# HKU-BAL/ClairS-TO

Measured on AMD Instinct MI355X. Metric: candidate sites/sec (pileup-tensor + AFF/NEG inference) at 1/2/4/8 MI355X, higher is better.
Workload: dtype f32; 1 GPU; ONT 50x synthetic pileups, SNV (K=4), 1M-site job cut into 4096-site chunks (BASELINE.json configs[1]); step = featurize(AFF+NEG) + CvT + BiGRU + posterior on one chunk; batch=4096, chunks_resident_per_gpu=16, min_bq_aff=20, pack_bytes_per_chunk=28614435, parallelism=sites sharded, 1 rank/GPU, weights=seeded random init (no pretrained weights offline)

## Files before the change

### clairs_to_amd/csrc/cvt_block.h

```cpp
#pragma once
#include "cvt_gemm.h"

namespace cto {

__host__ __device__ constexpr int emb_ps(int cin) { return cin > 0 ? ((cin - 4 + 15) / 16) * 16 + 4 : 0; }
__host__ __device__ constexpr int emb_kch(int cin) { return (3 * emb_ps(cin) + 15) / 16; }

template <int C, int W, int WKV, int TS, bool FOLD = false, int ECIN = 0>
struct CvtBlockGeom {
    static_assert(!FOLD || C <= 64, "folding pays only where C <= dim_head");
    static constexpr int R = TS * W, RKV = TS * WKV;
    static constexpr int MT = (R + 15) / 16, MTKV = (RKV + 15) / 16;
    static constexpr int AW = FOLD ? C : 64;
    static constexpr int RS = C + 4, QS = AW + 4, HC = (4 * C < 128 ? 4 * C : 128), US = HC + 4;
    static constexpr int KV_FLOATS = FOLD ? 0 : MTKV * 16 * QS;
    static constexpr int OFF_Y = 0;
    static constexpr int OFF_YKV = OFF_Y + MT * 16 * RS;
    static constexpr int OFF_Q = OFF_YKV + MTKV * 16 * RS;
    static constexpr int OFF_K = OFF_Q + MT * 16 * QS;
    static constexpr int OFF_V = OFF_K + KV_FLOATS;
    static constexpr int OFF_END = OFF_V + KV_FLOATS;
    static constexpr int SCRATCH = OFF_END - OFF_YKV;
    static constexpr int U_FLOATS = MT * 16 * US;
    static constexpr int emb_floats(int cin) { return (MT * 32 + 4) * emb_ps(cin); }
    static constexpr int TOTAL_BLK = OFF_END + (U_FLOATS > SCRATCH ? U_FLOATS - SCRATCH : 0);
    static constexpr int TOTAL_EMB = FOLD && ECIN > 0 ? OFF_YKV + emb_floats(ECIN) : 0;
    static constexpr int TOTAL = TOTAL_BLK > TOTAL_EMB ? TOTAL_BLK : TOTAL_EMB;
    static constexpr size_t LDS_BYTES = size_t(TOTAL) * sizeof(float);
    static constexpr int TMP_FLOATS = OFF_END - OFF_Q;
    static constexpr int ALIAS = TOTAL - OFF_YKV;
    static constexpr int KCH1 = (W * RS + 15) / 16;
    static constexpr bool HEAD_OK = (TS == 16) && (64 + head_lds_floats(6) <= ALIAS);
};

// ... 49 lines not shown
                                                const BPreS<ColOwn<N>::NTW>& pre,
                                                f32x4 (&acc)[MSplit<MTx, ColOwn<N>::MSPLIT>::MTG][ColOwn<N>::NTW], int j, int kg) {
    using S = MSplit<MTx, ColOwn<N>::MSPLIT>;
    constexpr int NTW = ColOwn<N>::NTW;
    const float* A0 = A + sp.mbase * 16 * lda;
    if (ColOwn<N>::MSPLIT == 1 || sp.mcount == S::MTG) {
        gemm_lds_split<S::MTG, NTW, KCH, F16>(A0, lda, klo, wrow, pre, acc, j, kg);
    } else if constexpr (S::LAST > 0) {
        if (sp.mcount == S::LAST) {
            f32x4 (&sub)[S::LAST][NTW] = reinterpret_cast<f32x4 (&)[S::LAST][NTW]>(acc);
            gemm_lds_split<S::LAST, NTW, KCH, F16>(A0, lda, klo, wrow, pre, sub, j, kg);
        }
    }
}

template <int C, int W, int WKV, int TS, bool FOLD = false, int ECIN = 0>
__host__ __device__ constexpr int cvt_blocks_per_cu() {
    using G = CvtBlockGeom<C, W, WKV, TS, FOLD, ECIN>;
    return G::LDS_BYTES * 3 <= 160 * 1024 && !FOLD ? 3 : (G::LDS_BYTES * 2 <= 160 * 1024 ? 2 : 1);
}

template <int N>
__device__ __forceinline__ float rowN_sum(float v) {
    static_assert(N == 4 || N == 8 || N == 16, "a quad, half a DPP row or a DPP row");
    v += dpp_mov<0xB1>(v);
    v += dpp_mov<0x4E>(v);
    if constexpr (N >= 8) v += dpp_mov<0x141>(v);
    if constexpr (N >= 16) v += dpp_mov<0x140>(v);
    return v;
}

template <int C, int W, int WKV, int TS, int CIN, bool HEAD, int SPLIT = 0, bool FOLD = false>
__global__ __launch_bounds__(CVT_BLOCK_THREADS, (2 * cvt_blocks_per_cu<C, W, WKV, TS, FOLD, FOLD ? CIN : 0>())) void k_cvt_block(float* __restrict__ h, CvtStageParams sp,
                                                                                                                  HeadTailParams hp, int heads, int B) {
    using G = CvtBlockGeom<C, W, WKV, TS, FOLD, FOLD ? CIN : 0>;
    static_assert(!FOLD || SPLIT == 0, "the folded matrices exist in fp32 only");
    constexpr bool SP = SPLIT != 0, F16 = SPLIT == 1;
    static_assert(!SP || (C % 64 == 0 && MT_EXACT<C, W, WKV, TS>()), "split GEMMs: 32-wide k chunks, 16-byte LayerNorm pieces, no pad rows");
    using WPtr = std::conditional_t<SP, const unsigned short*, const float*>;
    static_assert(CIN == 0 || G::emb_floats(CIN) <= G::ALIAS, "stage input tile does not fit the free LDS");
    static_assert(!HEAD || G::HEAD_OK, "classifier tail needs a 16-site tile and room for its scratch");
    static_assert(G::MT * 16 * G::RS <= G::TMP_FLOATS, "LayerNorm staging tile does not fit the q|k|v region");
    constexpr int NT = CVT_BLOCK_THREADS, NWV = CVT_WAVES;
    constexpr int R = G::R, MT = G::MT, MTKV = G::MTKV, RKV = G::RKV, RS = G::RS, QS = G::QS, HC = G::HC, US = G::US, AW = G::AW;
    static_assert(C % 16 == 0 && C <= 128 && NT % C == 0, "channel count must be 16, 32, 64 or 128");
    using OC = ColOwn<C>;
    using OQ = ColOwn<AW>;
    using OKV = ColOwn<128>;
    using OF = ColOwn<HC>;
    constexpr int MGC = MSplit<MT, OC::MSPLIT>::MTG, MGQ = MSplit<MT, OQ::MSPLIT>::MTG, MGF = MSplit<MT, OF::MSPLIT>::MTG;
    constexpr int NTC = OC::NTW, NTF = OF::NTW;
    static_assert(OQ::NTW == 1 && OKV::NTW == 1 && OKV::MSPLIT == 1, "q / kv tiles: one column tile per wave");
    extern __shared__ __attribute__((aligned(16))) float smem[];
    float* sy = smem + G::OFF_Y;
    float* sykv = smem + G::OFF_YKV;
    float* sq = smem + G::OFF_Q;
    float* sk = smem + G::OFF_K;
    float* sv = smem + G::OFF_V;
    float* stmp = smem + G::OFF_Q;
    float* su = smem + G::OFF_YKV;

    const int tid = threadIdx.x, lane = tid & 63, wave = tid >> 6, j = lane & 15, kg = lane >> 4;
    const TileSpan spc = tile_span<C, MT>(wave), spq = tile_span<AW, MT>(wave), spf = tile_span<HC, MT>(wave);
    const int site0 = blockIdx.x * TS;
    const int nsite = min(TS, B - site0);
    const int rows_valid = nsite * W;
    const int inner = heads * AW;
    float* hg = h + int64_t(site0) * W * C;
    int nstamp = 0;
    long long* const prof = sp.blk[0].prof;
    auto stamp = [&]() { if (prof && blockIdx.x == 0 && tid == 0 && nstamp < 250) prof[nstamp++] = clock64(); };
    stamp();
    const CvtBlockParams& pe = sp.blk[0];


    constexpr int KE_ = CIN > 0 ? emb_kch(CIN) : 1;
    const float* we_r[NTC];
    BPre<NTC> pre_e;
    if constexpr (CIN > 0) {
#pragma unroll
        for (int nt = 0; nt < NTC; ++nt) we_r[nt] = pe.wembp + int64_t(spc.tile0 + nt) * (KE_ * FRAG_CS) + 4 * lane;
        pre_e = prefetch_b<NTC, KE_>(we_r);
// ... 158 lines not shown
                if (mt < spc.mcount) {
#pragma unroll
                    for (int r = 0; r < 4; ++r) sy[((spc.mbase + mt) * 16 + 4 * kg + r) * RS + col] = acc_e[mt][nt][r] + bv;
                }
        }
        lds_barrier();
        for (int i = tid; i < (MTKV * 16 - RKV) * RS; i += NT) sykv[RKV * RS + i] = 0.f;
        layer_norm(sy, sy, pe.lng, pe.lnb, std::false_type{});
        lds_barrier();
    }

    f32x4 acc_f[MGC][NTC];
    for (int bi = 0; bi < sp.nblk; ++bi) {
    const CvtBlockParams& p = sp.blk[bi];
    stamp();
    f32x4 acc_o[MGC][NTC];
#pragma unroll
    for (int nt = 0; nt < NTC; ++nt) {
        const int col = (spc.tile0 + nt) * 16 + j;
        const float bv = p.bo[col];
#pragma unroll
        for (int mt = 0; mt < MGC; ++mt) {
            const int row0 = (spc.mbase + (mt < spc.mcount ? mt : 0)) * 16 + 4 * kg;
            if (bi == 0) {
#pragma unroll
                for (int r = 0; r < 4; ++r) acc_o[mt][nt][r] = sy[(row0 + r) * RS + col] + bv;
            } else {
#pragma unroll
                for (int r = 0; r < 4; ++r) acc_o[mt][nt][r] = acc_f[mt][nt][r] + bv;
            }
        }
    }
    layer_norm(sy, stmp, p.n0g, p.n0b, std::false_type{});
    lds_barrier();
    stamp();

#if CTO_CVT_ABL != 2
    {
        constexpr int NSLOT = NT / C;
        constexpr int PG = NSLOT > TS ? NSLOT / TS : 1;
        constexpr int SL = PG > 1 ? TS : NSLOT, NIT = (TS + SL - 1) / SL;
        constexpr int WQ = (W + PG - 1) / PG, WK = (WKV + PG - 1) / PG;
        const int c = tid % C, slot = tid / C, pg = slot / SL, s0 = slot - pg * SL;
        const int wlo = pg * WQ, whi = min(W, wlo + WQ), klo = pg * WK, khi = min(WKV, klo + WK);
        const float q0 = p.dwq[c * 3], q1 = p.dwq[c * 3 + 1], q2 = p.dwq[c * 3 + 2];
        const float k0 = p.dwkv[c * 3], k1 = p.dwkv[c * 3 + 1], k2 = p.dwkv[c * 3 + 2];
// ... 27 lines not shown
                    if constexpr (SP) put_split1<F16>(sykv + (s * WKV + wo) * RS, C, c, (d - km) * ki * kw + kb);
                    else sykv[(s * WKV + wo) * RS + c] = (d - km) * ki * kw + kb;
                }
            }
        }
    }
#endif
    lds_barrier();

    stamp();
    auto frag = [&](const float* w, const unsigned short* ws, int tile, int kch, int c0) -> WPtr {
        if constexpr (SP) return ws + (int64_t(tile) * kch + c0) * SPLIT_CS + 8 * lane;
        else return w + (int64_t(tile) * kch + c0) * FRAG_CS + 4 * lane;
    };
    constexpr int KD = SP ? 32 : 16;
    auto q_rows = [&](int hh, WPtr (&wr)[1]) { wr[0] = frag(p.wq, p.wq_s, hh * (AW / 16) + spq.tile0, C / KD, 0); };
    auto o_rows = [&](int hh, WPtr (&wr)[NTC]) {
#pragma unroll
        for (int nt = 0; nt < NTC; ++nt) wr[nt] = frag(p.wo, p.wo_s, spc.tile0 + nt, inner / KD, hh * (AW / KD));
    };
    auto w1_rows = [&](int cc, WPtr (&wr)[NTF]) {
#pragma unroll
        for (int nt = 0; nt < NTF; ++nt) wr[nt] = frag(p.w1, p.w1_s, cc * (HC / 16) + spf.tile0 + nt, C / KD, 0);
    };
    auto w2_rows = [&](int cc, WPtr (&wr)[NTC]) {
#pragma unroll
        for (int nt = 0; nt < NTC; ++nt) wr[nt] = frag(p.w2, p.w2_s, spc.tile0 + nt, 4 * C / KD, cc * (HC / KD));
    };
    WPtr wq_r[1];
    q_rows(0, wq_r);
    auto pre_q = prefetch_b<1, C / KD>(wq_r);
    for (int hh = 0; hh < heads; ++hh) {
        const int wn = wave & 3;
        WPtr wkv1_r[1] = {frag(p.wkv, p.wkv_s, (wave < 4 ? 0 : inner / 16) + hh * 4 + wn, C / KD, 0)};
        decltype(prefetch_b<1, C / KD>(wkv1_r)) pre_kv1;
        if constexpr (!FOLD) pre_kv1 = prefetch_b<1, C / KD>(wkv1_r);
        {
            f32x4 aq[MGQ][1];
#pragma unroll
            for (int mt = 0; mt < MGQ; ++mt) aq[mt][0] = f32x4{0.f, 0.f, 0.f, 0.f};
            if constexpr (SP) gemm_span_split<64, MT, C / 32, F16>(spq, sy, RS, C, wq_r, pre_q, aq, j, kg);
            else gemm_span<AW, MT, C / 16>(spq, sy, RS, wq_r, pre_q, aq, j, kg);
// ... 68 lines not shown
                }
            }
        }
#endif
        if (hh + 1 < heads) {
            q_rows(hh + 1, wq_r);
            pre_q = prefetch_b<1, C / KD>(wq_r);
        }
        lds_barrier();
        stamp();
        if constexpr (SP) gemm_span_split<C, MT, 2, F16>(spc, sq, QS, 64, wo_r, pre_o, acc_o, j, kg);
        else gemm_span<C, MT, AW / 16>(spc, sq, QS, wo_r, pre_o, acc_o, j, kg);
        lds_barrier();
        stamp();
    }

    WPtr w1_r[NTF];
    w1_rows(0, w1_r);
    auto pre_w1 = prefetch_b<NTF, C / KD>(w1_r);

#pragma unroll
    for (int nt = 0; nt < NTC; ++nt) {
        const int col = (spc.tile0 + nt) * 16 + j;
        const float bv = p.b2[col];
#pragma unroll
        for (int mt = 0; mt < MGC; ++mt) {
            if (mt < spc.mcount) {
#pragma unroll
                for (int r = 0; r < 4; ++r) stmp[((spc.mbase + mt) * 16 + 4 * kg + r) * RS + col] = acc_o[mt][nt][r];
            }
#pragma unroll
            for (int r = 0; r < 4; ++r) acc_f[mt][nt][r] = acc_o[mt][nt][r] + bv;
        }
    }
    lds_barrier();

    stamp();
    layer_norm(stmp, sy, p.n1g, p.n1b, std::bool_constant<SP>{});
    lds_barrier();
    stamp();

    for (int cc = 0; cc < 4 * C / HC; ++cc) {
        WPtr w2_r[NTC];
        w2_rows(cc, w2_r);
        const auto pre_w2 = prefetch_b<NTC, HC / KD>(w2_r);
        {
            f32x4 au[MGF][NTF];
#pragma unroll
            for (int mt = 0; mt < MGF; ++mt)
#pragma unroll
// ... 82 lines not shown
```

### clairs_to_amd/csrc/models.hip

```cpp
#include <cmath>
#include <cstdlib>
#include <cstring>
#include <map>
#include <memory>
#include <string>
#include <vector>
#include "common.h"
#include "nn_kernels.h"
#include "cvt_block.h"

using namespace cto;

int launch_gru_layer1(hipStream_t s, const float* x, const float* Wf, const float* bias, float* out, int64_t B);
int launch_gru_layer1_raw(hipStream_t s, const int16_t* x_raw, const int32_t* site_info, int which, int min_rescale_cov, const float* Wf,
                          const float* bias, float* out, int64_t B);
int launch_gru_layer2_fc1_split(hipStream_t s, const float* x, const void* Wp, const float* bias, const void* Fp, float* fc1_part,
                                int64_t B, bool f16, const float* scale5);
int launch_gru_layer1_split(hipStream_t s, const float* x, const void* Wp, const float* bias, float* out, int64_t B, bool f16,
                            const float* scale5);
int launch_gru_layer2_fc1(hipStream_t s, const float* x, const float* Wf, const float* bias, const float* fc1f, float* fc1_part, int64_t B);


struct cto_weights {
    std::map<std::string, std::vector<float>> t;
// ... 23 lines not shown
        if (rc != CTO_OK) return rc;
        CTO_HIP(hipMemcpy(p, v.data(), v.size() * sizeof(float), hipMemcpyHostToDevice));
        *out = static_cast<float*>(p);
        return CTO_OK;
    }
};

struct HeadDev {
    float *w1 = nullptr, *b1 = nullptr;
    float* w1p = nullptr;
    float *w2 = nullptr, *b2 = nullptr;
    float *w3 = nullptr, *b3 = nullptr;
    int k1 = 0;
};

struct BlockDev {
    float *n0g, *n0b, *dwq, *bnq, *wq, *dwkv, *bnkv, *wkv, *wo, *bo, *n1g, *n1b, *w1, *b1, *w2, *b2;
    float *wq_f = nullptr, *wkv_f = nullptr, *wo_f = nullptr, *w1_f = nullptr, *w2_f = nullptr;
    float *mq_f = nullptr, *mo_f = nullptr;
    float *wq_s = nullptr, *wkv_s = nullptr, *wo_s = nullptr, *w1_s = nullptr, *w2_s = nullptr;
};

struct StageDev {
    int cin, c, win, w, wkv, heads, inner;
    float *wemb, *bemb, *lng, *lnb;
    float* wembp = nullptr;
    std::vector<BlockDev> blocks;
};

}

struct cto_model {
    int device = -1;
    int kind = 0;
// ... 3 lines not shown
    float *gb1 = nullptr, *gb2 = nullptr;
    float *gw1f = nullptr, *gw2f = nullptr, *f1f = nullptr;
    float *gw1_split = nullptr, *gw2_split = nullptr, *f1_split = nullptr;
    bool split_f16 = false;
    float split_sc1[5] = {1.f, 1.f, 1.f, 1.f, 1.f}, split_sc2[5] = {1.f, 1.f, 1.f, 1.f, 1.f};
    int cvt_split = 0;
    HeadDev head;
    int64_t macs = 0;
    int64_t ws_B = 0;
    std::vector<void*> ws_ptrs;
    float* b_xexp = nullptr;
    int64_t xexp_B = 0;
    bool fuse_blocks = true;
    bool fuse_embed = true;
    bool fuse_head = true;
    bool fold = true;
    bool prof = false;
    bool prof_all = false;
    std::vector<std::pair<hipEvent_t, hipEvent_t>> prof_ev;
    std::vector<std::pair<hipEvent_t, hipEvent_t>> prof_ev1;
    int64_t prof_macs = 0;
    float *b_h = nullptr, *b_t = nullptr, *b_yq = nullptr, *b_ykv = nullptr, *b_q = nullptr, *b_kv = nullptr,
          *b_o = nullptr, *b_u = nullptr, *b_slab = nullptr, *b_h2 = nullptr;
    ~cto_model() {
        if (b_xexp) (void)hipFree(b_xexp);
        for (void* p : ws_ptrs) (void)hipFree(p);
        for (auto& e : prof_ev) { (void)hipEventDestroy(e.first); (void)hipEventDestroy(e.second); }
        for (auto& e : prof_ev1) { (void)hipEventDestroy(e.first); (void)hipEventDestroy(e.second); }
    }
};

// ... 168 lines not shown
        return rc;
    return launch_head(m, s, m->b_slab, S, B, logits);
}

struct RawIn { const int16_t* x; const int32_t* site_info; int which, min_rescale_cov; };

struct BlockExtra {
    const float* xin = nullptr;
    const RawIn* raw = nullptr;
    const StageDev* st = nullptr;
    const HeadDev* head = nullptr;
    float* logits = nullptr;
    int n_out = 0;
};

template <int C, int W, int WKV, int TS, int CIN, bool HEAD, int SPLIT = 0, bool FOLD = false>
int launch_cvt_block(hipStream_t s, float* h, const BlockDev* blocks, int nblk, int heads, int64_t B, const BlockExtra& ex) {
    using G = CvtBlockGeom<C, W, WKV, TS, FOLD, FOLD ? CIN : 0>;
    static_assert(G::LDS_BYTES <= 160 * 1024, "fused CvT block does not fit the 160 KB LDS of a gfx950 CU");
    static bool attr_set = false;
    if (!attr_set) {
        CTO_HIP(hipFuncSetAttribute(reinterpret_cast<const void*>(&k_cvt_block<C, W, WKV, TS, CIN, HEAD, SPLIT, FOLD>),
                                    hipFuncAttributeMaxDynamicSharedMemorySize, int(G::LDS_BYTES)));
        attr_set = true;
    }
    static long long* prof_buf = nullptr;
    static const bool prof_on = [] { const char* e = getenv("CTO_BLOCK_PROF"); return e && e[0] == '1'; }();
    if (prof_on && !prof_buf) CTO_HIP(hipMalloc(reinterpret_cast<void**>(&prof_buf), 256 * sizeof(long long)));
    if (prof_on) CTO_HIP(hipMemsetAsync(prof_buf, 0, 256 * sizeof(long long), s));
    CvtStageParams sp{};
    sp.nblk = nblk;
    for (int i = 0; i < nblk; ++i) {
        const BlockDev& b = blocks[i];
        if (FOLD) CTO_REQUIRE(b.mq_f && b.mo_f, CTO_EINVAL, "folded CvT block without folded weights");
        sp.blk[i] = CvtBlockParams{b.n0g, b.n0b, b.dwq, b.bnq, FOLD ? b.mq_f : b.wq_f, b.dwkv, b.bnkv, FOLD ? nullptr : b.wkv_f, FOLD ? b.mo_f : b.wo_f, b.bo, b.n1g, b.n1b, b.w1_f, b.b1, b.w2_f, b.b2,
                                   prof_on ? prof_buf : nullptr, nullptr, nullptr, nullptr, nullptr, nullptr, nullptr, nullptr,
                                   nullptr, nullptr, nullptr, nullptr, nullptr};
        if (SPLIT != 0) {
            CTO_REQUIRE(b.wq_s && b.wkv_s && b.wo_s && b.w1_s && b.w2_s, CTO_EINVAL, "split CvT block without split weights");
            CvtBlockParams& p = sp.blk[i];
            p.wq_s = reinterpret_cast<const unsigned short*>(b.wq_s); p.wkv_s = reinterpret_cast<const unsigned short*>(b.wkv_s);
            p.wo_s = reinterpret_cast<const unsigned short*>(b.wo_s); p.w1_s = reinterpret_cast<const unsigned short*>(b.w1_s);
            p.w2_s = reinterpret_cast<const unsigned short*>(b.w2_s);
        }
    }
    HeadTailParams hp{};
    if (CIN > 0) {
        CvtBlockParams& p = sp.blk[0];
        p.xin = ex.xin; p.wembp = ex.st->wembp; p.bemb = ex.st->bemb; p.lng = ex.st->lng; p.lnb = ex.st->lnb;
        if (ex.raw) { p.xraw = reinterpret_cast<const short*>(ex.raw->x); p.xinfo = ex.raw->site_info; p.xwhich = ex.raw->which; p.xcov = ex.raw->min_rescale_cov; }
// ... 5 lines not shown
    }
    hipLaunchKernelGGL((k_cvt_block<C, W, WKV, TS, CIN, HEAD, SPLIT, FOLD>), dim3(unsigned(cdiv(B, TS))), dim3(CVT_BLOCK_THREADS), G::LDS_BYTES,
                       s, h, sp, hp, heads, int(B));
    CTO_HIP(hipGetLastError());
    if (prof_on) {
        long long hst[256];
        CTO_HIP(hipStreamSynchronize(s));
        CTO_HIP(hipMemcpy(hst, prof_buf, sizeof(hst), hipMemcpyDeviceToHost));
        fprintf(stderr, "k_cvt_block<%d,%d,%d,%d,%d,%d,%d,%d> x%d stamps:", C, W, WKV, TS, CIN, int(HEAD), SPLIT, int(FOLD), nblk);
        for (int i = 1; i < 256 && hst[i]; ++i) fprintf(stderr, " %lld", hst[i] - hst[i - 1]);
        fprintf(stderr, "\n");
    }
    return CTO_OK;
}

constexpr bool cvt_fold_geom(int c) { return c <= 64; }

template <int C, int W, int WKV, int TS, int CIN, int SPLIT, bool FOLD = false>
int dispatch_block_kind(hipStream_t s, float* h, const BlockDev* blocks, int nblk, int heads, int64_t B, const BlockExtra& ex, bool embed, bool head) {
    if constexpr (FOLD) {
        return embed ? launch_cvt_block<C, W, WKV, TS, CIN, false, 0, true>(s, h, blocks, nblk, heads, B, ex)
                     : launch_cvt_block<C, W, WKV, TS, 0, false, 0, true>(s, h, blocks, nblk, heads, B, ex);
    }
    if constexpr (C == 128 && CvtBlockGeom<C, W, WKV, TS>::HEAD_OK) {
        if (head) return embed ? launch_cvt_block<C, W, WKV, TS, CIN, true, SPLIT>(s, h, blocks, nblk, heads, B, ex)
                               : launch_cvt_block<C, W, WKV, TS, 0, true, SPLIT>(s, h, blocks, nblk, heads, B, ex);
    }
    return embed ? launch_cvt_block<C, W, WKV, TS, CIN, false, SPLIT>(s, h, blocks, nblk, heads, B, ex)
                 : launch_cvt_block<C, W, WKV, TS, 0, false, SPLIT>(s, h, blocks, nblk, heads, B, ex);
}
template <int C, int W, int WKV, int TS, int CIN>
int dispatch_block(hipStream_t s, float* h, const BlockDev* blocks, int nblk, int heads, int64_t B, const BlockExtra& ex, bool embed, bool head,
                   int split, bool fold) {
    if constexpr (C % 64 == 0 && MT_EXACT<C, W, WKV, TS>()) {
        if (split == 1) return dispatch_block_kind<C, W, WKV, TS, CIN, 1>(s, h, blocks, nblk, heads, B, ex, embed, head);
        if (split == 2) return dispatch_block_kind<C, W, WKV, TS, CIN, 2>(s, h, blocks, nblk, heads, B, ex, embed, head);
    }
    if constexpr (cvt_fold_geom(C)) {
        if (fold && blocks->mq_f) return dispatch_block_kind<C, W, WKV, TS, CIN, 0, true>(s, h, blocks, nblk, heads, B, ex, embed, head);
    }
    return dispatch_block_kind<C, W, WKV, TS, CIN, 0>(s, h, blocks, nblk, heads, B, ex, embed, head);
}
#ifndef CTO_CVT_TS1
#define CTO_CVT_TS1 8
#endif
#ifndef CTO_CVT_TS2
#define CTO_CVT_TS2 16
#endif
#ifndef CTO_CVT_TS3
#define CTO_CVT_TS3 16
#endif
struct FusedGeom { int c, w, wkv, ts, cin; };
const FusedGeom* fused_geom(const StageDev& st) {
    static const FusedGeom G[4] = {{128, 5, 3, CTO_CVT_TS3, 64}, {64, 9, 5, CTO_CVT_TS2, 16}, {16, 17, 9, CTO_CVT_TS1, 34}, {32, 17, 9, CTO_CVT_TS1, 34}};
    for (const FusedGeom& g : G)
        if (st.c == g.c && st.w == g.w && st.wkv == g.wkv) return &g;
    return nullptr;
}
bool can_fuse_embed(const StageDev& st) { const FusedGeom* g = fused_geom(st); return g && g->cin == st.cin && st.wembp; }
bool can_fuse_head(const StageDev& st, const HeadDev& hd) { const FusedGeom* g = fused_geom(st); return g && g->ts == 16 && g->c == 128 && hd.w1p; }

int try_fused_blocks(hipStream_t s, const StageDev& st, const BlockDev* b, int nblk, float* h, int64_t B, const BlockExtra& ex, bool embed,
                     bool head, int split, bool fold) {
    int rc = CTO_OK;
    if (!b->wq_s) split = 0;
    if (split) fold = false;
    if (st.c == 128 && st.w == 5 && st.wkv == 3) rc = dispatch_block<128, 5, 3, CTO_CVT_TS3, 64>(s, h, b, nblk, st.heads, B, ex, embed, head, split, fold);
    else if (st.c == 64 && st.w == 9 && st.wkv == 5) rc = dispatch_block<64, 9, 5, CTO_CVT_TS2, 16>(s, h, b, nblk, st.heads, B, ex, embed, head, split, fold);
    else if (st.c == 16 && st.w == 17 && st.wkv == 9) rc = dispatch_block<16, 17, 9, CTO_CVT_TS1, 34>(s, h, b, nblk, st.heads, B, ex, embed, head, split, fold);
    else if (st.c == 32 && st.w == 17 && st.wkv == 9) rc = dispatch_block<32, 17, 9, CTO_CVT_TS1, 34>(s, h, b, nblk, st.heads, B, ex, embed, head, split, fold);
    else return 0;
    return rc == CTO_OK ? 1 : rc;
}

int cvt_forward(cto_model* m, const float* x, int64_t B, float* logits, hipStream_t s, const RawIn* raw = nullptr) {
    int rc;
    const float* in = x;
    for (int si = 0; si < 3; ++si) {
        const StageDev& st = m->st[si];
        const int M = int(B) * st.w, Mkv = int(B) * st.wkv, C = st.c;
        float* hbuf = (si & 1) ? m->b_h2 : m->b_h;
// ... 186 lines not shown
    std::vector<uint16_t> fr(size_t(ntiles) * kch32 * 2 * 64 * 8);
    for (int t = 0; t < ntiles; ++t)
        for (int c = 0; c < kch32; ++c)
            for (int lane = 0; lane < 64; ++lane) {
                const int j = lane & 15, kg = lane >> 4;
                const float* src = v->data() + size_t(t * 16 + j) * K + c * 32 + kg * 8;
                if (f16)
                    for (int e = 0; e < 8; ++e)
                        CTO_REQUIRE(std::fabs(src[e]) < 60000.f, CTO_EUNSUPPORTED, "CTO_CVT_SPLIT=f16: weight %s holds %g, outside the f16 range",
                                    name.c_str(), double(src[e]));
                const size_t u = ((size_t(t) * kch32 + c) * 2) * 64;
                put_split8(&fr[(u + lane) * 8], &fr[(u + 64 + lane) * 8], src, 8, f16);
            }
    return upload_halves(fr, a, out);
}
int upload_folded(const cto_weights* w, const std::string& P, int C, int heads, Arena& a, float** mq, float** mo) {
    int rc = CTO_OK;
    const int inner = 64 * heads;
    GETW(wq, P + ".0.fn.to_q.net.2.weight", int64_t(inner) * C);
    GETW(wkv, P + ".0.fn.to_kv.net.2.weight", int64_t(2) * inner * C);
    GETW(wo, P + ".0.fn.to_out.0.weight", int64_t(C) * inner);
    const float* wk = wkv->data();
    const float* wv = wkv->data() + size_t(inner) * C;
    std::vector<float> q(size_t(heads) * C * C), o(size_t(C) * heads * C);
    for (int hh = 0; hh < heads; ++hh)
        for (int x = 0; x < C; ++x)
            for (int y = 0; y < C; ++y) {
                double sq = 0.0, so = 0.0;
                for (int d = 0; d < 64; ++d) {
                    const size_t r = size_t(hh) * 64 + d;
                    sq += double(wk[r * C + x]) * double((*wq)[r * C + y]);
                    so += double(wv[r * C + y]) * double((*wo)[size_t(x) * inner + r]);
                }
                q[(size_t(hh) * C + x) * C + y] = float(sq);
                o[size_t(x) * heads * C + size_t(hh) * C + y] = float(so);
            }
    if ((rc = a.upload(pack_fragments(q.data(), heads * C / 16, C / 16), mq)) != CTO_OK) return rc;
    return a.upload(pack_fragments(o.data(), C / 16, heads * C / 16), mo);
}
int upload_fragments(const cto_weights* w, const std::string& name, int ntiles, int kch, Arena& a, float** out) {
    int rc = CTO_OK;
    GETW(v, name, int64_t(ntiles) * 16 * kch * 16);
    return a.upload(pack_fragments(v->data(), ntiles, kch), out);
}

int pack_gru_split(const cto_weights* w, const std::string& base, int kin, int kp, int H, const std::vector<float>* fc1, bool f16,
                   int log2_sx, Arena& a, float** Wout, float** Fout, float* scale5) {
    const int NB = H / 64, NX = kp / 32, NH = H / 32, NC = NX + NH, T = 33;
    int rc = CTO_OK;
    std::vector<uint16_t> W(size_t(2) * 4 * NC * NB * 6 * 64 * 8), F(fc1 ? size_t(2) * T * 4 * NH * 4 * 64 * 8 : 0);
    float w_ih_scale = 1.f, w_hh_scale = 1.f, f_scale = 1.f;
    scale5[0] = scale5[1] = scale5[2] = scale5[3] = scale5[4] = 1.f;
    if (f16) {
// ... 123 lines not shown
                (rc = upload_named(w, P + ".0.fn.to_out.0.bias", C, a, &b.bo)) ||
                (rc = upload_named(w, P + ".1.norm.g", C, a, &b.n1g)) || (rc = upload_named(w, P + ".1.norm.b", C, a, &b.n1b)) ||
                (rc = upload_named(w, P + ".1.fn.net.0.weight", int64_t(4) * C * C, a, &b.w1)) ||
                (rc = upload_named(w, P + ".1.fn.net.0.bias", 4 * C, a, &b.b1)) ||
                (rc = upload_named(w, P + ".1.fn.net.3.weight", int64_t(4) * C * C, a, &b.w2)) ||
                (rc = upload_named(w, P + ".1.fn.net.3.bias", C, a, &b.b2)))
                return fail(rc);
            const int NI = st.inner / 16, NC16 = C / 16;
            if (C % 16 == 0 &&
                ((rc = upload_fragments(w, P + ".0.fn.to_q.net.2.weight", NI, NC16, a, &b.wq_f)) ||
                (rc = upload_fragments(w, P + ".0.fn.to_kv.net.2.weight", 2 * NI, NC16, a, &b.wkv_f)) ||
                (rc = upload_fragments(w, P + ".0.fn.to_out.0.weight", NC16, NI, a, &b.wo_f)) ||
                (rc = upload_fragments(w, P + ".1.fn.net.0.weight", 4 * NC16, NC16, a, &b.w1_f)) ||
                 (rc = upload_fragments(w, P + ".1.fn.net.3.weight", NC16, 4 * NC16, a, &b.w2_f))))
                return fail(rc);
            if (fused_geom(st) && cvt_fold_geom(C) && (rc = upload_folded(w, P, C, st.heads, a, &b.mq_f, &b.mo_f))) return fail(rc);
            if (m->cvt_split && C % 64 == 0) {
                const bool f16 = m->cvt_split == 1;
                if ((rc = upload_split_fragments(w, P + ".0.fn.to_q.net.2.weight", NI, C / 32, f16, a, &b.wq_s)) ||
                    (rc = upload_split_fragments(w, P + ".0.fn.to_kv.net.2.weight", 2 * NI, C / 32, f16, a, &b.wkv_s)) ||
                    (rc = upload_split_fragments(w, P + ".0.fn.to_out.0.weight", NC16, st.inner / 32, f16, a, &b.wo_s)) ||
                    (rc = upload_split_fragments(w, P + ".1.fn.net.0.weight", 4 * NC16, C / 32, f16, a, &b.w1_s)) ||
                    (rc = upload_split_fragments(w, P + ".1.fn.net.3.weight", NC16, 4 * C / 32, f16, a, &b.w2_s)))
                    return fail(rc);
            }
            st.blocks.push_back(b);
            macs += int64_t(st.w) * C * st.inner + int64_t(st.wkv) * C * 2 * st.inner + int64_t(st.w) * st.inner * C +
                    int64_t(st.w) * 8 * C * C + int64_t(2) * st.heads * st.w * st.wkv * 64 +
                    int64_t(3) * C * (st.w + st.wkv);
        }
        cin = C;
// ... 11 lines not shown
        if (C3 == 128 && W3 == 5) {
            using G = CvtBlockGeom<128, 5, 3, 16>;
            const int KP = G::KCH1 * 16;
            std::vector<float> vp(size_t(128) * KP, 0.f);
            for (int n = 0; n < 128; ++n)
                for (int ww = 0; ww < W3; ++ww)
                    for (int c = 0; c < C3; ++c) vp[size_t(n) * KP + ww * G::RS + c] = v[size_t(n) * k1 + ww * C3 + c];
            if ((rc = a.upload(pack_fragments(vp.data(), 8, G::KCH1), &m->head.w1p))) return fail(rc);
        }
    }
    macs += int64_t(k1) * 128 + int64_t(m->n_out) * (128 * 128 + 256);
    m->macs = macs;
    if (const char* e = getenv("CTO_CVT_UNFUSED")) m->fuse_blocks = !(e[0] == '1');
    if (const char* e = getenv("CTO_CVT_NO_EMBED_FUSE")) m->fuse_embed = !(e[0] == '1');
    if (const char* e = getenv("CTO_CVT_NO_HEAD_FUSE")) m->fuse_head = !(e[0] == '1');
    if (const char* e = getenv("CTO_CVT_FOLD")) m->fold = !(e[0] == '0');
    *out = m.release();
    return CTO_OK;
}

extern "C" int cto_bigru_create(const cto_weights* w, int n_out, cto_model** out) {
    return cto_bigru_create_ex(w, n_out, CTO_SPLIT_ENV, out);
}

extern "C" int cto_bigru_create_ex(const cto_weights* w, int n_out, int split_mode, cto_model** out) {
    CTO_REQUIRE(w && out, CTO_EINVAL, "cto_bigru_create: null argument");
    CTO_REQUIRE(split_mode >= CTO_SPLIT_ENV && split_mode <= CTO_SPLIT_BF16, CTO_EINVAL, "cto_bigru_create_ex: split_mode %d", split_mode);
    CTO_REQUIRE(n_out == 4 || n_out == 6, CTO_EINVAL, "n_out must be 4 or 6");
    std::unique_ptr<cto_model> m(new cto_model());
    CTO_HIP(hipGetDevice(&m->device));
    m->kind = 1;
// ... 145 lines not shown
```

Measured before the change: 2.231 million sites/s.

## Fold attention weights into key/value side for C=64 and C=128 CvT stages

Adds a KV-side algebraic fold: Wq^T·Wk and Wv·Wo are premultiplied per head on the host, so keys and values are projected into C-wide space. The kernel then computes attention directly against the LayerNormed input and accumulates into the residual in registers. This removes the separate Q and output projection GEMMs, and it becomes the default for the 64- and 128-channel stages (the 16-channel stage keeps the query-side fold). In exchange, the KV GEMM grows to 2C columns per head and extra weights are uploaded, which may cost more FLOPs when heads*64 is not much larger than C.

```diff
diff --git a/clairs_to_amd/csrc/cvt_block.h b/clairs_to_amd/csrc/cvt_block.h
--- a/clairs_to_amd/csrc/cvt_block.h
+++ b/clairs_to_amd/csrc/cvt_block.h
@@ -6,18 +6,20 @@
 __host__ __device__ constexpr int emb_ps(int cin) { return cin > 0 ? ((cin - 4 + 15) / 16) * 16 + 4 : 0; }
 __host__ __device__ constexpr int emb_kch(int cin) { return (3 * emb_ps(cin) + 15) / 16; }
 
-template <int C, int W, int WKV, int TS, bool FOLD = false, int ECIN = 0>
+constexpr int FOLD_NONE = 0, FOLD_Q = 1, FOLD_KV = 2;
+template <int C, int W, int WKV, int TS, int FOLD = FOLD_NONE, int ECIN = 0>
 struct CvtBlockGeom {
-    static_assert(!FOLD || C <= 64, "folding pays only where C <= dim_head");
+    static_assert(FOLD != FOLD_Q || C <= 64, "folding on the query side pays only where C <= dim_head");
     static constexpr int R = TS * W, RKV = TS * WKV;
     static constexpr int MT = (R + 15) / 16, MTKV = (RKV + 15) / 16;
     static constexpr int AW = FOLD ? C : 64;
-    static constexpr int RS = C + 4, QS = AW + 4, HC = (4 * C < 128 ? 4 * C : 128), US = HC + 4;
+    static constexpr int RS = C + 4, QS = FOLD == FOLD_KV ? 2 * C + 4 : AW + 4, HC = (4 * C < 128 ? 4 * C : 128), US = HC + 4;
     static constexpr int KV_FLOATS = FOLD ? 0 : MTKV * 16 * QS;
+    static constexpr int Q_FLOATS = FOLD == FOLD_KV ? (MTKV * QS > MT * RS ? MTKV * 16 * QS : MT * 16 * RS) : MT * 16 * QS;
     static constexpr int OFF_Y = 0;
     static constexpr int OFF_YKV = OFF_Y + MT * 16 * RS;
     static constexpr int OFF_Q = OFF_YKV + MTKV * 16 * RS;
-    static constexpr int OFF_K = OFF_Q + MT * 16 * QS;
+    static constexpr int OFF_K = OFF_Q + Q_FLOATS;
     static constexpr int OFF_V = OFF_K + KV_FLOATS;
     static constexpr int OFF_END = OFF_V + KV_FLOATS;
     static constexpr int SCRATCH = OFF_END - OFF_YKV;
@@ -97,7 +99,7 @@
     }
 }
 
-template <int C, int W, int WKV, int TS, bool FOLD = false, int ECIN = 0>
+template <int C, int W, int WKV, int TS, int FOLD = FOLD_NONE, int ECIN = 0>
 __host__ __device__ constexpr int cvt_blocks_per_cu() {
     using G = CvtBlockGeom<C, W, WKV, TS, FOLD, ECIN>;
     return G::LDS_BYTES * 3 <= 160 * 1024 && !FOLD ? 3 : (G::LDS_BYTES * 2 <= 160 * 1024 ? 2 : 1);
@@ -113,12 +115,12 @@
     return v;
 }
 
-template <int C, int W, int WKV, int TS, int CIN, bool HEAD, int SPLIT = 0, bool FOLD = false>
+template <int C, int W, int WKV, int TS, int CIN, bool HEAD, int SPLIT = 0, int FOLD = FOLD_NONE>
 __global__ __launch_bounds__(CVT_BLOCK_THREADS, (2 * cvt_blocks_per_cu<C, W, WKV, TS, FOLD, FOLD ? CIN : 0>())) void k_cvt_block(float* __restrict__ h, CvtStageParams sp,
                                                                                                                   HeadTailParams hp, int heads, int B) {
     using G = CvtBlockGeom<C, W, WKV, TS, FOLD, FOLD ? CIN : 0>;
     static_assert(!FOLD || SPLIT == 0, "the folded matrices exist in fp32 only");
-    constexpr bool SP = SPLIT != 0, F16 = SPLIT == 1;
+    constexpr bool SP = SPLIT != 0, F16 = SPLIT == 1, KVF = FOLD == FOLD_KV;
     static_assert(!SP || (C % 64 == 0 && MT_EXACT<C, W, WKV, TS>()), "split GEMMs: 32-wide k chunks, 16-byte LayerNorm pieces, no pad rows");
     using WPtr = std::conditional_t<SP, const unsigned short*, const float*>;
     static_assert(CIN == 0 || G::emb_floats(CIN) <= G::ALIAS, "stage input tile does not fit the free LDS");
@@ -138,17 +140,14 @@
     float* sy = smem + G::OFF_Y;
     float* sykv = smem + G::OFF_YKV;
     float* sq = smem + G::OFF_Q;
-    float* sk = smem + G::OFF_K;
-    float* sv = smem + G::OFF_V;
     float* stmp = smem + G::OFF_Q;
     float* su = smem + G::OFF_YKV;
 
     const int tid = threadIdx.x, lane = tid & 63, wave = tid >> 6, j = lane & 15, kg = lane >> 4;
-    const TileSpan spc = tile_span<C, MT>(wave), spq = tile_span<AW, MT>(wave), spf = tile_span<HC, MT>(wave);
+    const TileSpan spc = tile_span<C, MT>(wave), spf = tile_span<HC, MT>(wave);
     const int site0 = blockIdx.x * TS;
     const int nsite = min(TS, B - site0);
     const int rows_valid = nsite * W;
-    const int inner = heads * AW;
     float* hg = h + int64_t(site0) * W * C;
     int nstamp = 0;
     long long* const prof = sp.blk[0].prof;
@@ -337,7 +336,24 @@
     for (int bi = 0; bi < sp.nblk; ++bi) {
     const CvtBlockParams& p = sp.blk[bi];
     stamp();
-    f32x4 acc_o[MGC][NTC];
+    f32x4 acc_o[KVF ? 1 : MGC][NTC];
+    constexpr int NVK = C > 64 ? C / 64 : 1, LPK = C / (4 * NVK), RPK = NT / LPK, NPK = (MT * 16 + RPK - 1) / RPK;
+    static_assert(!KVF || (C % (4 * NVK) == 0 && (LPK == 4 || LPK == 8 || LPK == 16)), "attention lane groups: a quad, half a DPP row or a DPP row");
+    const int l4k = (tid % LPK) * 4, rowk = tid / LPK;
+    float4 ho[KVF ? NPK : 1][NVK];
+    if constexpr (KVF) {
+#pragma unroll
+        for (int u = 0; u < NVK; ++u) {
+            const float* bp = p.bo + l4k + 64 * u;
+            const float4 b4 = make_float4(bp[0], bp[1], bp[2], bp[3]);
+#pragma unroll
+            for (int q = 0; q < NPK; ++q) {
+                const int rr = min(q * RPK + rowk, MT * 16 - 1);
+                const float4 h4 = *reinterpret_cast<const float4*>(sy + rr * RS + l4k + 64 * u);
+                ho[q][u] = make_float4(h4.x + b4.x, h4.y + b4.y, h4.z + b4.z, h4.w + b4.w);
+            }
+        }
+    } else {
 #pragma unroll
     for (int nt = 0; nt < NTC; ++nt) {
         const int col = (spc.tile0 + nt) * 16 + j;
@@ -353,6 +369,7 @@
                 for (int r = 0; r < 4; ++r) acc_o[mt][nt][r] = acc_f[mt][nt][r] + bv;
             }
         }
+    }
     }
     layer_norm(sy, stmp, p.n0g, p.n0b, std::false_type{});
     lds_barrier();
@@ -410,11 +427,6 @@
         else return w + (int64_t(tile) * kch + c0) * FRAG_CS + 4 * lane;
     };
     constexpr int KD = SP ? 32 : 16;
-    auto q_rows = [&](int hh, WPtr (&wr)[1]) { wr[0] = frag(p.wq, p.wq_s, hh * (AW / 16) + spq.tile0, C / KD, 0); };
-    auto o_rows = [&](int hh, WPtr (&wr)[NTC]) {
-#pragma unroll
-        for (int nt = 0; nt < NTC; ++nt) wr[nt] = frag(p.wo, p.wo_s, spc.tile0 + nt, inner / KD, hh * (AW / KD));
-    };
     auto w1_rows = [&](int cc, WPtr (&wr)[NTF]) {
 #pragma unroll
         for (int nt = 0; nt < NTF; ++nt) wr[nt] = frag(p.w1, p.w1_s, cc * (HC / 16) + spf.tile0 + nt, C / KD, 0);
@@ -422,6 +434,113 @@
     auto w2_rows = [&](int cc, WPtr (&wr)[NTC]) {
 #pragma unroll
         for (int nt = 0; nt < NTC; ++nt) wr[nt] = frag(p.w2, p.w2_s, spc.tile0 + nt, 4 * C / KD, cc * (HC / KD));
+    };
+    if constexpr (KVF) {
+        using OK = ColOwn<2 * C>;
+        constexpr int NTK = OK::NTW, MGK = MSplit<MTKV, OK::MSPLIT>::MTG;
+        const TileSpan spk = tile_span<2 * C, MTKV>(wave);
+        float* skv = sq;
+        auto kv_rows = [&](int hh, WPtr (&wr)[NTK]) {
+#pragma unroll
+            for (int nt = 0; nt < NTK; ++nt) wr[nt] = frag(p.wkv, p.wkv_s, hh * (2 * C / 16) + spk.tile0 + nt, C / KD, 0);
+        };
+        WPtr wk_r[NTK];
+        kv_rows(0, wk_r);
+        auto pre_k = prefetch_b<NTK, C / KD>(wk_r);
+        float4 qv[NPK][NVK];
+#pragma unroll
+        for (int q = 0; q < NPK; ++q) {
+            const int row = q * RPK + rowk, rr = row < R ? row : 0;
+#pragma unroll
+            for (int u = 0; u < NVK; ++u) qv[q][u] = *reinterpret_cast<const float4*>(sy + rr * RS + l4k + 64 * u);
+        }
+        for (int hh = 0; hh < heads; ++hh) {
+            {
+                f32x4 ak[MGK][NTK];
+#pragma unroll
+                for (int mt = 0; mt < MGK; ++mt)
+#pragma unroll
+                    for (int nt = 0; nt < NTK; ++nt) ak[mt][nt] = f32x4{0.f, 0.f, 0.f, 0.f};
+                gemm_span<2 * C, MTKV, C / 16>(spk, sykv, RS, wk_r, pre_k, ak, j, kg);
+#pragma unroll
+                for (int nt = 0; nt < NTK; ++nt)
+#pragma unroll
+                    for (int mt = 0; mt < MGK; ++mt)
+                        if (mt < spk.mcount) {
+#pragma unroll
+                            for (int r = 0; r < 4; ++r) skv[((spk.mbase + mt) * 16 + 4 * kg + r) * QS + (spk.tile0 + nt) * 16 + j] = ak[mt][nt][r];
+                        }
+            }
+            if (hh + 1 < heads) {
+                kv_rows(hh + 1, wk_r);
+                pre_k = prefetch_b<NTK, C / KD>(wk_r);
+            }
+            lds_barrier();
+            stamp();
+#if CTO_CVT_ABL != 2
+#pragma unroll
+            for (int q = 0; q < NPK; ++q) {
+                const int row = q * RPK + rowk, rr = row < R ? row : 0;
+                const float* kb = skv + (rr / W) * WKV * QS + l4k;
+                float4 kv[WKV][NVK], vv[WKV][NVK];
+#pragma unroll
+                for (int jj = 0; jj < WKV; ++jj)
+#pragma unroll
+                    for (int u = 0; u < NVK; ++u) kv[jj][u] = *reinterpret_cast<const float4*>(kb + jj * QS + 64 * u);
+                float sc[WKV];
+#pragma unroll
+                for (int jj = 0; jj < WKV; ++jj) {
+                    sc[jj] = fmaf(qv[q][0].w, kv[jj][0].w, fmaf(qv[q][0].z, kv[jj][0].z, fmaf(qv[q][0].y, kv[jj][0].y, qv[q][0].x * kv[jj][0].x)));
+#pragma unroll
+                    for (int u = 1; u < NVK; ++u)
+                        sc[jj] = fmaf(qv[q][u].w, kv[jj][u].w, fmaf(qv[q][u].z, kv[jj][u].z, fmaf(qv[q][u].y, kv[jj][u].y, fmaf(qv[q][u].x, kv[jj][u].x, sc[jj]))));
+                }
+                if constexpr (WKV > 5) {
+#pragma unroll
+                    for (int jj = 0; jj < WKV; ++jj) asm volatile("" : "+v"(sc[jj]));
+                    __builtin_amdgcn_sched_barrier(0);
+                }
+#pragma unroll
+                for (int jj = 0; jj < WKV; ++jj)
+#pragma unroll
+                    for (int u = 0; u < NVK; ++u) vv[jj][u] = *reinterpret_cast<const float4*>(kb + jj * QS + C + 64 * u);
+#pragma unroll
+                for (int jj = 0; jj < WKV; ++jj) sc[jj] = rowN_sum<LPK>(sc[jj]);
+                float mx = sc[0];
+#pragma unroll
+                for (int jj = 1; jj < WKV; ++jj) mx = fmaxf(mx, sc[jj]);
+                float sum = 0.f;
+#pragma unroll
+                for (int jj = 0; jj < WKV; ++jj) { sc[jj] = exp_le0((sc[jj] - mx) * 0.125f); sum += sc[jj]; }
+                float inv = rcp_fast(sum);
+                inv = fmaf(fmaf(-sum, inv, 1.0f), inv, inv);
+                if (row >= R) inv = 0.f;
+#pragma unroll
+                for (int jj = 0; jj < WKV; ++jj) {
+                    const float pj = sc[jj] * inv;
+#pragma unroll
+                    for (int u = 0; u < NVK; ++u) {
+                        ho[q][u].x = fmaf(pj, vv[jj][u].x, ho[q][u].x); ho[q][u].y = fmaf(pj, vv[jj][u].y, ho[q][u].y);
+                        ho[q][u].z = fmaf(pj, vv[jj][u].z, ho[q][u].z); ho[q][u].w = fmaf(pj, vv[jj][u].w, ho[q][u].w);
+                    }
+                }
+#pragma unroll
+                for (int u = 0; u < NVK; ++u) asm volatile("" : "+v"(ho[q][u].x), "+v"(ho[q][u].y), "+v"(ho[q][u].z), "+v"(ho[q][u].w));
+                if ((q + 1) % (WKV <= 5 ? 2 : 1) == 0) __builtin_amdgcn_sched_barrier(0);
+            }
+#endif
+            lds_barrier();
+            stamp();
+        }
+    } else {
+    const TileSpan spq = tile_span<AW, MT>(wave);
+    const int inner = heads * AW;
+    float* sk = smem + G::OFF_K;
+    float* sv = smem + G::OFF_V;
+    auto q_rows = [&](int hh, WPtr (&wr)[1]) { wr[0] = frag(p.wq, p.wq_s, hh * (AW / 16) + spq.tile0, C / KD, 0); };
+    auto o_rows = [&](int hh, WPtr (&wr)[NTC]) {
+#pragma unroll
+        for (int nt = 0; nt < NTC; ++nt) wr[nt] = frag(p.wo, p.wo_s, spc.tile0 + nt, inner / KD, hh * (AW / KD));
     };
     WPtr wq_r[1];
     q_rows(0, wq_r);
@@ -520,26 +639,44 @@
         lds_barrier();
         stamp();
     }
+    }
 
     WPtr w1_r[NTF];
     w1_rows(0, w1_r);
     auto pre_w1 = prefetch_b<NTF, C / KD>(w1_r);
 
+    if constexpr (KVF) {
+#pragma unroll
+        for (int q = 0; q < NPK; ++q) {
+            const int row = q * RPK + rowk;
+            if (row < MT * 16) {
+#pragma unroll
+                for (int u = 0; u < NVK; ++u) *reinterpret_cast<float4*>(stmp + row * RS + l4k + 64 * u) = ho[q][u];
+            }
+        }
+        lds_barrier();
+    }
 #pragma unroll
     for (int nt = 0; nt < NTC; ++nt) {
         const int col = (spc.tile0 + nt) * 16 + j;
         const float bv = p.b2[col];
 #pragma unroll
         for (int mt = 0; mt < MGC; ++mt) {
-            if (mt < spc.mcount) {
-#pragma unroll
-                for (int r = 0; r < 4; ++r) stmp[((spc.mbase + mt) * 16 + 4 * kg + r) * RS + col] = acc_o[mt][nt][r];
-            }
-#pragma unroll
-            for (int r = 0; r < 4; ++r) acc_f[mt][nt][r] = acc_o[mt][nt][r] + bv;
-        }
-    }
-    lds_barrier();
+            if constexpr (KVF) {
+                const int row0 = (spc.mbase + (mt < spc.mcount ? mt : 0)) * 16 + 4 * kg;
+#pragma unroll
+                for (int r = 0; r < 4; ++r) acc_f[mt][nt][r] = stmp[(row0 + r) * RS + col] + bv;
+            } else {
+                if (mt < spc.mcount) {
+#pragma unroll
+                    for (int r = 0; r < 4; ++r) stmp[((spc.mbase + mt) * 16 + 4 * kg + r) * RS + col] = acc_o[mt][nt][r];
+                }
+#pragma unroll
+                for (int r = 0; r < 4; ++r) acc_f[mt][nt][r] = acc_o[mt][nt][r] + bv;
+            }
+        }
+    }
+    if constexpr (!KVF) lds_barrier();
 
     stamp();
     layer_norm(stmp, sy, p.n1g, p.n1b, std::bool_constant<SP>{});
diff --git a/clairs_to_amd/csrc/models.hip b/clairs_to_amd/csrc/models.hip
--- a/clairs_to_amd/csrc/models.hip
+++ b/clairs_to_amd/csrc/models.hip
@@ -61,10 +61,13 @@
     int k1 = 0;
 };
 
+enum { CVT_FOLD_OFF = 0, CVT_FOLD_DEFAULT = 1, CVT_FOLD_QSIDE = 2, CVT_FOLD_KVSIDE = 3 };
+
 struct BlockDev {
     float *n0g, *n0b, *dwq, *bnq, *wq, *dwkv, *bnkv, *wkv, *wo, *bo, *n1g, *n1b, *w1, *b1, *w2, *b2;
     float *wq_f = nullptr, *wkv_f = nullptr, *wo_f = nullptr, *w1_f = nullptr, *w2_f = nullptr;
     float *mq_f = nullptr, *mo_f = nullptr;
+    float* mkv_f = nullptr;
     float *wq_s = nullptr, *wkv_s = nullptr, *wo_s = nullptr, *w1_s = nullptr, *w2_s = nullptr;
 };
 
@@ -98,7 +101,7 @@
     bool fuse_blocks = true;
     bool fuse_embed = true;
     bool fuse_head = true;
-    bool fold = true;
+    int fold = CVT_FOLD_DEFAULT;
     bool prof = false;
     bool prof_all = false;
     std::vector<std::pair<hipEvent_t, hipEvent_t>> prof_ev;
@@ -297,7 +300,7 @@
     int n_out = 0;
 };
 
-template <int C, int W, int WKV, int TS, int CIN, bool HEAD, int SPLIT = 0, bool FOLD = false>
+template <int C, int W, int WKV, int TS, int CIN, bool HEAD, int SPLIT = 0, int FOLD = FOLD_NONE>
 int launch_cvt_block(hipStream_t s, float* h, const BlockDev* blocks, int nblk, int heads, int64_t B, const BlockExtra& ex) {
     using G = CvtBlockGeom<C, W, WKV, TS, FOLD, FOLD ? CIN : 0>;
     static_assert(G::LDS_BYTES <= 160 * 1024, "fused CvT block does not fit the 160 KB LDS of a gfx950 CU");
@@ -315,8 +318,10 @@
     sp.nblk = nblk;
     for (int i = 0; i < nblk; ++i) {
         const BlockDev& b = blocks[i];
-        if (FOLD) CTO_REQUIRE(b.mq_f && b.mo_f, CTO_EINVAL, "folded CvT block without folded weights");
-        sp.blk[i] = CvtBlockParams{b.n0g, b.n0b, b.dwq, b.bnq, FOLD ? b.mq_f : b.wq_f, b.dwkv, b.bnkv, FOLD ? nullptr : b.wkv_f, FOLD ? b.mo_f : b.wo_f, b.bo, b.n1g, b.n1b, b.w1_f, b.b1, b.w2_f, b.b2,
+        if (FOLD == FOLD_Q) CTO_REQUIRE(b.mq_f && b.mo_f, CTO_EINVAL, "folded CvT block without folded weights");
+        if (FOLD == FOLD_KV) CTO_REQUIRE(b.mkv_f, CTO_EINVAL, "folded CvT block without folded weights");
+        sp.blk[i] = CvtBlockParams{b.n0g, b.n0b, b.dwq, b.bnq, FOLD == FOLD_Q ? b.mq_f : (FOLD ? nullptr : b.wq_f), b.dwkv, b.bnkv,
+                                   FOLD == FOLD_KV ? b.mkv_f : (FOLD ? nullptr : b.wkv_f), FOLD == FOLD_Q ? b.mo_f : (FOLD ? nullptr : b.wo_f), b.bo, b.n1g, b.n1b, b.w1_f, b.b1, b.w2_f, b.b2,
                                    prof_on ? prof_buf : nullptr, nullptr, nullptr, nullptr, nullptr, nullptr, nullptr, nullptr,
                                    nullptr, nullptr, nullptr, nullptr, nullptr};
         if (SPLIT != 0) {
@@ -352,13 +357,27 @@
     return CTO_OK;
 }
 
-constexpr bool cvt_fold_geom(int c) { return c <= 64; }
-
-template <int C, int W, int WKV, int TS, int CIN, int SPLIT, bool FOLD = false>
+constexpr bool cvt_fold_q_geom(int c) { return c <= 64; }
+constexpr int cvt_fold_default(int c) {
+    return c == 128 ? FOLD_KV
+         : c == 64  ? FOLD_KV
+                    : FOLD_Q;
+}
+constexpr int cvt_fold_kind(int mode, int c) {
+    return mode == CVT_FOLD_OFF ? FOLD_NONE : mode == CVT_FOLD_QSIDE ? (cvt_fold_q_geom(c) ? FOLD_Q : FOLD_NONE) : mode == CVT_FOLD_KVSIDE ? FOLD_KV : cvt_fold_default(c);
+}
+
+template <int C, int W, int WKV, int TS, int CIN, int SPLIT, int FOLD = FOLD_NONE>
 int dispatch_block_kind(hipStream_t s, float* h, const BlockDev* blocks, int nblk, int heads, int64_t B, const BlockExtra& ex, bool embed, bool head) {
-    if constexpr (FOLD) {
-        return embed ? launch_cvt_block<C, W, WKV, TS, CIN, false, 0, true>(s, h, blocks, nblk, heads, B, ex)
-                     : launch_cvt_block<C, W, WKV, TS, 0, false, 0, true>(s, h, blocks, nblk, heads, B, ex);
+    if constexpr (FOLD != FOLD_NONE) {
+        static_assert(SPLIT == 0, "the folded matrices exist in fp32 only");
+        if constexpr (C == 128 && CvtBlockGeom<C, W, WKV, TS>::HEAD_OK) {
+            static_assert(CvtBlockGeom<C, W, WKV, TS, FOLD, CIN>::HEAD_OK && CvtBlockGeom<C, W, WKV, TS, FOLD, 0>::HEAD_OK, "no room for the classifier tail");
+            if (head) return embed ? launch_cvt_block<C, W, WKV, TS, CIN, true, 0, FOLD>(s, h, blocks, nblk, heads, B, ex)
+                                   : launch_cvt_block<C, W, WKV, TS, 0, true, 0, FOLD>(s, h, blocks, nblk, heads, B, ex);
+        }
+        return embed ? launch_cvt_block<C, W, WKV, TS, CIN, false, 0, FOLD>(s, h, blocks, nblk, heads, B, ex)
+                     : launch_cvt_block<C, W, WKV, TS, 0, false, 0, FOLD>(s, h, blocks, nblk, heads, B, ex);
     }
     if constexpr (C == 128 && CvtBlockGeom<C, W, WKV, TS>::HEAD_OK) {
         if (head) return embed ? launch_cvt_block<C, W, WKV, TS, CIN, true, SPLIT>(s, h, blocks, nblk, heads, B, ex)
@@ -369,14 +388,16 @@
 }
 template <int C, int W, int WKV, int TS, int CIN>
 int dispatch_block(hipStream_t s, float* h, const BlockDev* blocks, int nblk, int heads, int64_t B, const BlockExtra& ex, bool embed, bool head,
-                   int split, bool fold) {
+                   int split, int fold) {
     if constexpr (C % 64 == 0 && MT_EXACT<C, W, WKV, TS>()) {
         if (split == 1) return dispatch_block_kind<C, W, WKV, TS, CIN, 1>(s, h, blocks, nblk, heads, B, ex, embed, head);
         if (split == 2) return dispatch_block_kind<C, W, WKV, TS, CIN, 2>(s, h, blocks, nblk, heads, B, ex, embed, head);
     }
-    if constexpr (cvt_fold_geom(C)) {
-        if (fold && blocks->mq_f) return dispatch_block_kind<C, W, WKV, TS, CIN, 0, true>(s, h, blocks, nblk, heads, B, ex, embed, head);
-    }
+    const int kind = cvt_fold_kind(fold, C);
+    if constexpr (cvt_fold_q_geom(C)) {
+        if (kind == FOLD_Q && blocks->mq_f) return dispatch_block_kind<C, W, WKV, TS, CIN, 0, FOLD_Q>(s, h, blocks, nblk, heads, B, ex, embed, head);
+    }
+    if (kind == FOLD_KV && blocks->mkv_f) return dispatch_block_kind<C, W, WKV, TS, CIN, 0, FOLD_KV>(s, h, blocks, nblk, heads, B, ex, embed, head);
     return dispatch_block_kind<C, W, WKV, TS, CIN, 0>(s, h, blocks, nblk, heads, B, ex, embed, head);
 }
 #ifndef CTO_CVT_TS1
@@ -399,10 +420,10 @@
 bool can_fuse_head(const StageDev& st, const HeadDev& hd) { const FusedGeom* g = fused_geom(st); return g && g->ts == 16 && g->c == 128 && hd.w1p; }
 
 int try_fused_blocks(hipStream_t s, const StageDev& st, const BlockDev* b, int nblk, float* h, int64_t B, const BlockExtra& ex, bool embed,
-                     bool head, int split, bool fold) {
+                     bool head, int split, int fold) {
     int rc = CTO_OK;
     if (!b->wq_s) split = 0;
-    if (split) fold = false;
+    if (split) fold = CVT_FOLD_OFF;
     if (st.c == 128 && st.w == 5 && st.wkv == 3) rc = dispatch_block<128, 5, 3, CTO_CVT_TS3, 64>(s, h, b, nblk, st.heads, B, ex, embed, head, split, fold);
     else if (st.c == 64 && st.w == 9 && st.wkv == 5) rc = dispatch_block<64, 9, 5, CTO_CVT_TS2, 16>(s, h, b, nblk, st.heads, B, ex, embed, head, split, fold);
     else if (st.c == 16 && st.w == 17 && st.wkv == 9) rc = dispatch_block<16, 17, 9, CTO_CVT_TS1, 34>(s, h, b, nblk, st.heads, B, ex, embed, head, split, fold);
@@ -619,7 +640,7 @@
             }
     return upload_halves(fr, a, out);
 }
-int upload_folded(const cto_weights* w, const std::string& P, int C, int heads, Arena& a, float** mq, float** mo) {
+int upload_folded(const cto_weights* w, const std::string& P, int C, int heads, Arena& a, float** mq, float** mo, float** mkv) {
     int rc = CTO_OK;
     const int inner = 64 * heads;
     GETW(wq, P + ".0.fn.to_q.net.2.weight", int64_t(inner) * C);
@@ -627,7 +648,7 @@
     GETW(wo, P + ".0.fn.to_out.0.weight", int64_t(C) * inner);
     const float* wk = wkv->data();
     const float* wv = wkv->data() + size_t(inner) * C;
-    std::vector<float> q(size_t(heads) * C * C), o(size_t(C) * heads * C);
+    std::vector<float> q(size_t(heads) * C * C), o(size_t(C) * heads * C), kv(size_t(heads) * 2 * C * C);
     for (int hh = 0; hh < heads; ++hh)
         for (int x = 0; x < C; ++x)
             for (int y = 0; y < C; ++y) {
@@ -639,9 +660,12 @@
                 }
                 q[(size_t(hh) * C + x) * C + y] = float(sq);
                 o[size_t(x) * heads * C + size_t(hh) * C + y] = float(so);
+                kv[(size_t(hh) * 2 * C + y) * C + x] = float(sq);
+                kv[(size_t(hh) * 2 * C + C + x) * C + y] = float(so);
             }
-    if ((rc = a.upload(pack_fragments(q.data(), heads * C / 16, C / 16), mq)) != CTO_OK) return rc;
-    return a.upload(pack_fragments(o.data(), C / 16, heads * C / 16), mo);
+    if (mq && (rc = a.upload(pack_fragments(q.data(), heads * C / 16, C / 16), mq)) != CTO_OK) return rc;
+    if (mo && (rc = a.upload(pack_fragments(o.data(), C / 16, heads * C / 16), mo)) != CTO_OK) return rc;
+    return a.upload(pack_fragments(kv.data(), heads * 2 * C / 16, C / 16), mkv);
 }
 int upload_fragments(const cto_weights* w, const std::string& name, int ntiles, int kch, Arena& a, float** out) {
     int rc = CTO_OK;
@@ -795,7 +819,8 @@
                 (rc = upload_fragments(w, P + ".1.fn.net.0.weight", 4 * NC16, NC16, a, &b.w1_f)) ||
                  (rc = upload_fragments(w, P + ".1.fn.net.3.weight", NC16, 4 * NC16, a, &b.w2_f))))
                 return fail(rc);
-            if (fused_geom(st) && cvt_fold_geom(C) && (rc = upload_folded(w, P, C, st.heads, a, &b.mq_f, &b.mo_f))) return fail(rc);
+            if (fused_geom(st) && (rc = upload_folded(w, P, C, st.heads, a, cvt_fold_q_geom(C) ? &b.mq_f : nullptr, cvt_fold_q_geom(C) ? &b.mo_f : nullptr, &b.mkv_f)))
+                return fail(rc);
             if (m->cvt_split && C % 64 == 0) {
                 const bool f16 = m->cvt_split == 1;
                 if ((rc = upload_split_fragments(w, P + ".0.fn.to_q.net.2.weight", NI, C / 32, f16, a, &b.wq_s)) ||
@@ -837,7 +862,10 @@
     if (const char* e = getenv("CTO_CVT_UNFUSED")) m->fuse_blocks = !(e[0] == '1');
     if (const char* e = getenv("CTO_CVT_NO_EMBED_FUSE")) m->fuse_embed = !(e[0] == '1');
     if (const char* e = getenv("CTO_CVT_NO_HEAD_FUSE")) m->fuse_head = !(e[0] == '1');
-    if (const char* e = getenv("CTO_CVT_FOLD")) m->fold = !(e[0] == '0');
+    if (const char* e = getenv("CTO_CVT_FOLD")) {
+        const std::string v(e);
+        m->fold = e[0] == '0' ? CVT_FOLD_OFF : v == "q" ? CVT_FOLD_QSIDE : v == "kv" ? CVT_FOLD_KVSIDE : CVT_FOLD_DEFAULT;
+    }
     *out = m.release();
     return CTO_OK;
 }
```

Result: faster. 2.282 million sites/s, median of 6 (+2.3%).
